# cornellius-gp/linear_operator

Measured on AMD Instinct MI355X. Metric: cg_member_matvecs_per_sec, higher is better.
Workload: dtype f32

## Files before the change

### linear_operator_amd/csrc/lo_rspace3.hip

```cpp
#include <algorithm>
#include <atomic>
#include <mutex>
#include <type_traits>
#include <stdlib.h>

#include "lo_device.h"
#include "lo_internal.h"
#include "lo_cg_onchip.h"
#include "lo_group_reduce.h"
#include "lo_cg_close.h"
#include "lo_f64_lanes.h"

namespace lo {

namespace {

typedef float f32x4 __attribute__((ext_vector_type(4)));
typedef __attribute__((address_space(1))) const f32x4 g_cf4;
typedef __attribute__((address_space(1))) const float g_cf;
typedef __attribute__((address_space(1))) float g_f;
typedef __attribute__((address_space(1))) const char g_cc;
template <class T>
__device__ __forceinline__ T* opaque_uniform(T* p) {
  asm volatile("" : "+s"(p));
  return p;
}

constexpr int R3_TPB = 256;
constexpr int R3_ROWS = 1024;

struct PeerOut {
  float* buf[7];
  int n;
  long long member_off;
};
PeerOut g_peer_out = {{nullptr, nullptr, nullptr, nullptr, nullptr, nullptr, nullptr}, 0, 0};
std::mutex g_peer_mu;

__host__ __device__ constexpr int r3_np(int RC) { return 2 * RC + 6; }

__device__ __forceinline__ unsigned xor4_dpp_u(unsigned x) {
  const int a = __builtin_amdgcn_update_dpp(0, (int)x, 0x104, 0xf, 0x5, false);
  return (unsigned)__builtin_amdgcn_update_dpp(a, (int)x, 0x114, 0xf, 0xa, false);
}
__device__ __forceinline__ double halve4_d(double lo, double hi, int lane) {
  const bool up = (lane & 4) != 0;
  const double keep = up ? hi : lo;
  const double send = up ? lo : hi;
  return keep + mk_d(xor4_dpp_u(lo_w(send)), xor4_dpp_u(hi_w(send)));
}

template <int CH>
__device__ __forceinline__ double rows_reduce_d(double (&p)[CH], int lane) {
  if constexpr (CH == 8) {
#pragma unroll
    for (int m = 0; m < 4; ++m) p[m] = halve4_d(p[m], p[m + 4], lane);
    p[0] = halve_pair_d<2>(p[0], p[2], lane);
    p[1] = halve_pair_d<2>(p[1], p[3], lane);
    return halve_pair_d<1>(p[0], p[1], lane);
  } else if constexpr (CH == 4) {
    p[0] = halve_pair_d<2>(p[0], p[2], lane);
    p[1] = halve_pair_d<2>(p[1], p[3], lane);
    return halve_pair_d<1>(p[0], p[1], lane);
  } else {
    return halve_pair_d<1>(p[0], p[1], lane);
  }
}

template <int RC, int GW>
__global__ __launch_bounds__(R3_TPB, 2) void k_cg_rspace3(OnchipArgs a, PeerOut po) {
  constexpr int CH = RC / 4;
  constexpr int RPI = 64 / CH;
  constexpr int NI = 256 / RPI;
  constexpr int NP = r3_np(RC);
  constexpr int MLD = RC + 2;
  constexpr int NH = RC / 2;
  constexpr int NG = 2 * GW * NP;
  __shared__ __attribute__((aligned(16))) float bst[4][256];
  __shared__ __attribute__((aligned(16))) float dst[4][256];
  __shared__ __attribute__((aligned(16))) double mat_s[3 * RC * MLD];
  __shared__ __attribute__((aligned(16))) double red[4][NP];
  __shared__ __attribute__((aligned(16))) double res[NP];
  __shared__ __attribute__((aligned(16))) double gv[4][32];
  __shared__ unsigned polw[GW > 1 ? NG : 2];
  const GroupPlace gp = group_place(GW, (int)gridDim.x / 8);
  if (!gp.active) return;
  const int grp = gp.grp, wig = gp.wig, ngroups = gp.ngroups;
  const int t = threadIdx.x, lane = t & 63, wave = t >> 6;
  const int wave_u = __builtin_amdgcn_readfirstlane(wave);
  unsigned long long* const gbase = a.gbuf + (size_t)grp * 2 * NG;
  unsigned tag = a.tag_base;
  bool same_xcd = false;
  const unsigned xcc = xcc_id();
  bool first = true;
  const int row0 = wig * R3_ROWS + 256 * wave_u;
  const int row0c = max(0, min(row0, a.N - 256));
  const bool di_full = a.dinv_mode == LO_DIAG_FULL;
  float* const bw = bst[wave_u];
  float* const dw = dst[wave_u];
  constexpr int NPF = 8;
  f32x4 pre[NPF];
  constexpr int NXT = NI - NPF;
  f32x4 nxt[NXT > 0 ? NXT : 1];
  auto request = [&](int64_t bm, int tl_, int i_lo, auto cnt, f32x4* dst) {
    const int ln_ = tl_ & 63, k_ = ln_ & (CH - 1), g_ = ln_ / CH;
    const unsigned loff = (unsigned)((g_ * RC + 4 * k_) * sizeof(float));
    g_cc* Cw = (g_cc*)(a.C + ((size_t)bm * a.N + row0c) * RC);
#pragma unroll
    for (int q = 0; q < decltype(cnt)::value / 8; ++q) {
      g_cc* bq = opaque_uniform(Cw + (i_lo + 8 * q + 4) * 1024);
#pragma unroll
      for (int i = 0; i < 8; ++i) dst[8 * q + i] = *(g_cf4*)(bq + loff + (i - 4) * 1024);
    }
  };
  int closed = 0;
  int64_t b = grp;
  {
    int tl0 = t;
    asm volatile("" : "+v"(tl0));
    if (b < a.B) {
      request(b, tl0, 0, std::integral_constant<int, NPF>{}, pre);
      request(b, tl0, NPF, std::integral_constant<int, NXT>{}, nxt);
    } else {
#pragma unroll
      for (int i = 0; i < NPF; ++i) pre[i] = (f32x4){0.f, 0.f, 0.f, 0.f};
    }
  }
  while (b < a.B) {
    const bool stamp = a.dbg && b == a.dbg_member && wig == 0 && t == 0;
    if (stamp) a.dbg[0] = wall_clock64();
    int drawn = 0;
    if (wig == 0 && t == 0) drawn = atomicAdd(a.next_member, 1);
    int tl = t;
    asm volatile("" : "+v"(tl));
    const int ln = tl & 63, k = ln & (CH - 1), g = ln / CH;
    f32x4 Cr[NI];
#pragma unroll
    for (int i = 0; i < NPF; ++i) Cr[i] = pre[i];
#pragma unroll
    for (int i = 0; i < NXT; ++i) Cr[NPF + i] = nxt[i];
    float bq4[4], dq4[4];
    {
      g_cf* bb_ = opaque_uniform((g_cf*)(a.rhs + (size_t)b * a.N + row0c));
      g_cf* dd_ = opaque_uniform((g_cf*)(di_full ? a.dinv + (size_t)b * a.N + row0c : a.dinv + b));
      const int lo_e = row0 - row0c, hi_e = max(0, min(256, a.N - row0c));
      const int dstride = di_full ? 1 : 0;
#pragma unroll
      for (int m = 0; m < 4; ++m) {
        const int e = ln + 64 * m;
        const bool own = e >= lo_e && e < hi_e;
        bq4[m] = own ? bb_[e] : 0.f;
        dq4[m] = own ? dd_[e * dstride] : 0.f;
      }
    }
    constexpr int NM = (3 * RC * RC / 2 + R3_TPB - 1) / R3_TPB;
    f32x4 mv[NM];
    {
      typedef __attribute__((address_space(1))) const f32x4 g_m4;
      const g_m4* src = (const g_m4*)(a.RSD + (size_t)b * 6 * RC * RC);
#pragma unroll
      for (int u = 0; u < NM; ++u) {
        const int e = min(tl + R3_TPB * u, 3 * RC * RC / 2 - 1);
        const int ms = e / (RC * RC / 2);
        const int mg = ms == 0 ? 0 : ms + 1;
        mv[u] = src[(size_t)mg * (RC * RC / 2) + (e - ms * (RC * RC / 2))];
      }
    }
    const double lam_mine = a.RSD[((size_t)b * 6 + 5) * RC * RC + min(ln & 31, RC - 1)];
#pragma unroll
    for (int m = 0; m < 4; ++m) {
      bw[ln + 64 * m] = bq4[m];
      dw[ln + 64 * m] = dq4[m];
    }
#pragma unroll
    for (int u = 0; u < NM; ++u) {
      const int e = tl + R3_TPB * u;
      if (e < 3 * RC * RC / 2) {
        const int mi = e / (RC / 2), jj = e % (RC / 2);
        *reinterpret_cast<f32x4*>(&mat_s[mi * MLD + 2 * jj]) = mv[u];
      }
    }
    __builtin_amdgcn_wave_barrier();
    if (stamp) a.dbg[1] = wall_clock64();

    {
      double aw[4] = {0.0, 0.0, 0.0, 0.0}, au[4] = {0.0, 0.0, 0.0, 0.0};
#pragma unroll
      for (int i0 = 0; i0 < NI; i0 += 4) {
#pragma unroll
        for (int i = i0; i < i0 + 4; ++i) {
          const int r = RPI * i + g;
          const double bb = (double)bw[r];
          const double bd = bb * (double)dw[r];
          const double c0 = (double)Cr[i].x, c1 = (double)Cr[i].y, c2 = (double)Cr[i].z, c3 = (double)Cr[i].w;
          aw[0] = fma(c0, bd, aw[0]); au[0] = fma(c0, bb, au[0]);
          aw[1] = fma(c1, bd, aw[1]); au[1] = fma(c1, bb, au[1]);
          aw[2] = fma(c2, bd, aw[2]); au[2] = fma(c2, bb, au[2]);
          aw[3] = fma(c3, bd, aw[3]); au[3] = fma(c3, bb, au[3]);
        }
        __builtin_amdgcn_sched_barrier(0);
      }
      double s_acc = 0.0, a_acc = 0.0, d2_acc = 0.0;
#pragma unroll
      for (int j = 0; j < 4; ++j) {
        const int rw = 64 * j + RPI * k + g;
        const double bb = (double)bw[rw], di = (double)dw[rw];
        s_acc = fma(bb, bb * di, s_acc);
        a_acc = fma(bb, bb, a_acc);
        d2_acc = fma(di, di, d2_acc);
      }
      double h0 = halve_pair_d<32>(aw[0], au[0], ln), h1 = halve_pair_d<32>(aw[1], au[1], ln);
      double h2 = halve_pair_d<32>(aw[2], au[2], ln), h3 = halve_pair_d<32>(aw[3], au[3], ln);
      h0 = halve_pair_d<16>(h0, h2, ln);
      h1 = halve_pair_d<16>(h1, h3, ln);
      double mine = halve_pair_d<8>(h0, h1, ln);
      if constexpr (CH <= 4) mine = bfly_add_d<4>(mine);
      if constexpr (CH <= 2) mine = bfly_add_d<2>(mine);
      const int comp = (((ln >> 4) & 1) << 1) | ((ln >> 3) & 1);
      const bool writer = (ln & 7 & ~(CH - 1)) == 0;
      if (writer) red[wave_u][((ln >> 5) ? RC : 0) + 4 * k + comp] = mine;
      const double ssum = wave_sum_fast_d(s_acc), asum = wave_sum_fast_d(a_acc), d2sum = wave_sum_fast_d(d2_acc);
      if (ln == 0) {
        red[wave_u][2 * RC] = ssum;
        red[wave_u][2 * RC + 1] = asum;
        red[wave_u][2 * RC + 2] = (wig == 0 && wave_u == 0) ? (double)(ngroups + drawn) : 0.0;
        red[wave_u][2 * RC + 3] = d2sum;
        unsigned xc = xcc;
        asm volatile("" : "+s"(xc));
        red[wave_u][2 * RC + 4] = (first && wave_u == 0) ? (double)xc : 0.0;
        red[wave_u][2 * RC + 5] = (first && wave_u == 0) ? (double)(xc * xc) : 0.0;
      }
    }
#pragma unroll
    for (int i = 0; i < NI; ++i) asm volatile("" : "+v"(Cr[i]));
    __builtin_amdgcn_sched_barrier(0);
    if (a.prefetch & 4) __builtin_amdgcn_s_setprio(3);
    {
      ++tag;
      int tt = (int)threadIdx.x;
      asm volatile("" : "+v"(tt));
      __syncthreads();
      if constexpr (GW == 1) {
        if (tt < NP) res[tt] = (red[0][tt] + red[1][tt]) + (red[2][tt] + red[3][tt]);
      } else {
        unsigned long long* slot = gbase + (size_t)(tag & 1u) * NG;
        if (tt < NP) {
          const double v = (red[0][tt] + red[1][tt]) + (red[2][tt] + red[3][tt]);
          unsigned long long* mine = slot + ((size_t)wig * NP + tt) * 2;
          granule_store(mine, granule_pack_bits(tag, lo_w(v)), same_xcd);
          granule_store(mine + 1, granule_pack_bits(tag, hi_w(v)), same_xcd);
        }
        constexpr int PER = (NG + R3_TPB - 1) / R3_TPB;
        constexpr int CKQ = PER < 8 ? PER : 8;
        unsigned spin = 0;
        bool lost = false;
#pragma unroll 1
        for (int q0 = 0; q0 < PER && !lost; q0 += CKQ) {
          unsigned long long x[CKQ];
          for (;;) {
            bool ok = true;
#pragma unroll
            for (int q = 0; q < CKQ; ++q) {
              const int idx = tt + R3_TPB * (q0 + q);
              x[q] = granule_load(slot + min(idx, NG - 1));
              ok = ok && (granule_tag(x[q]) == tag);
            }
            if (ok) break;
            if (poll_give_up(spin, a.err)) {
              lost = true;
              break;
            }
            __builtin_amdgcn_s_sleep(1);
          }
#pragma unroll
          for (int q = 0; q < CKQ; ++q) {
            const int idx = tt + R3_TPB * (q0 + q);
            if (idx < NG) polw[idx] = granule_bits(x[q]);
          }
        }
        __syncthreads();
        if (tt < NP) {
          double tot = 0.0;
#pragma unroll
          for (int w = 0; w < GW; ++w) tot += mk_d(polw[(w * NP + tt) * 2], polw[(w * NP + tt) * 2 + 1]);
          res[tt] = tot;
        }
      }
      __syncthreads();
    }
    if (GW > 1 && first) {
      unsigned xc = xcc;
      asm volatile("" : "+s"(xc));
      same_xcd = same_xcd_verdict(res[2 * RC + 4], res[2 * RC + 5], GW, xc, a.allow_l2_handoff);
    }
    first = false;
    if (stamp) a.dbg[2] = wall_clock64();
    const int64_t b_next = (int64_t)res[2 * RC + 2];
    {
      int tp = t;
      asm volatile("" : "+v"(tp));
      if (b_next < a.B) {
        request(b_next, tp, 0, std::integral_constant<int, NPF>{}, pre);
      } else {
#pragma unroll
        for (int i = 0; i < NPF; ++i) pre[i] = (f32x4){0.f, 0.f, 0.f, 0.f};
      }
    }
    if (a.prefetch & 1) __builtin_amdgcn_s_setprio(3);

    const int j = lane & 31, hf = lane >> 5;
    const bool live = j < RC;
    const int jr = live ? j : RC - 1;
    double yj = 0.0, xi = 0.0;
    float nrm;
    {
      double a0 = res[2 * RC + 1], s = res[2 * RC];
      const double d2 = res[2 * RC + 3];
      nrm = sqrtf((float)a0);
      const bool rhs_zero = nrm < a.eps;
      if (rhs_zero) nrm = 1.0f;
      const double inv = 1.0 / (double)nrm;
      const double w0 = live ? res[jr] * inv : 0.0, u0 = live ? res[RC + jr] * inv : 0.0;
      s *= inv * inv;
      a0 *= inv * inv;
      float sa = a.stop_after;
      asm volatile("" : "+s"(sa));
      const double sure_rz = 2.0 * (double)sa * (double)sa * sqrt(d2);
      auto own_row_dot = [&](const double* mrow, const double* vec) {
        double a0_ = 0.0, a1_ = 0.0;
#pragma unroll
        for (int q = 0; q < NH; q += 2) {
          const double2 xa = *reinterpret_cast<const double2*>(mrow + q);
          const double2 xx = *reinterpret_cast<const double2*>(vec + q);
          a0_ = fma(xa.x, xx.x, a0_);
          a1_ = fma(xa.y, xx.y, a1_);
        }
        double lo_, up_;
        halves_d(a0_ + a1_, lo_, up_);
        return lo_ + up_;
      };
      double* myv = gv[wave];
      if (hf == 0) myv[j] = w0;
      __builtin_amdgcn_wave_barrier();
      const double* row0m = mat_s + (size_t)jr * MLD + hf * NH;
      double c0 = own_row_dot(row0m, myv + hf * NH);
      double e0 = own_row_dot(row0m + (size_t)1 * RC * MLD, myv + hf * NH);
      const double* nrow = row0m + (size_t)2 * RC * MLD;
      const double* tucol = mat_s + (size_t)(1 * RC + hf * NH) * MLD + jr;
      c0 = live ? c0 : 0.0;
      e0 = live ? e0 : 0.0;
      double tau2 = s - lanes32_sum_d(c0 * e0);
      tau2 = tau2 > 0.0 ? tau2 : 0.0;
      const bool delicate = !rhs_zero && tau2 < 1e-2 * s;
      const double lam = live ? lam_mine : 1.0;
      long long ts_a = 0, ts_b = 0;
      if (stamp) ts_a = wall_clock64();
      double cj = c0, qj = 0.0, etaj = 0.0;
      double cp = 1.0, qp = 0.0, etap = 0.0;
      double rz = 0.0, pApE = 0.0, alpha = 0.0, beta = 0.0;
      float rn = 0.f, last_alpha = 0.f;
      bool conv = false;
      unsigned close_flags = 0u;
      const size_t bc = (size_t)b;
      const bool rec = wig == 0 && lane == 0;
      const int last_owner = (a.iters - 1) & 3;
      for (int kk = -1; kk < a.iters; ++kk) {
        if (kk >= 0) {
          last_alpha = (float)alpha;
          etaj = fma(alpha, qj, etaj);
          etap = fma(alpha, qp, etap);
          cj = fma(-alpha * lam, qj, cj);
          cp = fma(-alpha, qp, cp);
        }
        const double lc = lam * cj;
        const bool lo_h = hf == 0;
        const float inv_rz = __builtin_amdgcn_rcpf((float)rz);
        const double red2 = row16_sum_d(halve_pair_d<16>(lo_h ? cj * cj : lc * qj, lo_h ? lc * cj : 0.0, lane));
        const auto pick = [&](double v, int ln_) {
          return mk_d((unsigned)__builtin_amdgcn_readlane((int)lo_w(v), ln_),
                      (unsigned)__builtin_amdgcn_readlane((int)hi_w(v), ln_));
        };
        const double cc = pick(red2, 0), clc = pick(red2, 16), clq = pick(red2, 32);
        const double rzn = fma(cp * cp, tau2, cc);
        const bool sure = rzn > sure_rz;
        const bool rec_first = kk == 0 && a.close_gran == nullptr && wave == 0;
        const bool rec_last = kk == a.iters - 1 && wave == last_owner;
        const bool own = rec_first || rec_last || !sure;
        float rnn = 0.f;
        if (kk < 0) {
          const float s1f = (float)a0;
          rnn = __builtin_amdgcn_sqrtf(s1f < 0.f ? 0.f : s1f);
        } else if (own) {
          const double dl = fma(-cp, c0, cj);
          __builtin_amdgcn_wave_barrier();
          if (hf == 0) myv[j] = dl;
          __builtin_amdgcn_wave_barrier();
          double gj_;
          {
            double a0_ = 0.0, a1_ = 0.0;
#pragma unroll
            for (int q = 0; q < NH; q += 2) {
              const double2 dd = *reinterpret_cast<const double2*>(myv + hf * NH + q);
              a0_ = fma(tucol[(size_t)q * MLD], dd.x, a0_);
              a1_ = fma(tucol[(size_t)(q + 1) * MLD], dd.y, a1_);
            }
            double lo_, up_;
            halves_d(a0_ + a1_, lo_, up_);
            gj_ = live ? lo_ + up_ : 0.0;
          }
          __builtin_amdgcn_wave_barrier();
          if (hf == 0) myv[j] = gj_;
          __builtin_amdgcn_wave_barrier();
          const double nd = own_row_dot(nrow, myv + hf * NH);
          const double r2 = row16_sum_d(halve_pair_d<16>(gj_ * nd, gj_ * u0, lane));
          const double dnd = pick(r2, 0), dm = pick(r2, 16);
          const double s1 = fma(cp, fma(cp, a0, 2.0 * dm), dnd);
          const float s1f = (float)s1;
          rnn = __builtin_amdgcn_sqrtf(s1f < 0.f ? 0.f : s1f);
        }
        if (kk >= 0) {
          beta = ((float)rz < a.eps) ? 0.0 : (double)((float)rzn * inv_rz);
          if (rhs_zero) rnn = 0.f;
          rn = rnn;
          if (rec && (rec_first || rec_last)) a.resid_rec[(size_t)kk * a.B + bc] = rn;
        } else {
          beta = 0.0;
          rn = rnn;
          if (wig == 0 && t == 0) a.init_conv[bc] = (rn < a.stop_after) ? 1 : 0;
          close_flags = ((rn < a.stop_after) ? 1u : 0u) | (delicate ? 4u : 0u);
          if (delicate && rec && wave == 0) atomicOr(a.err + 4, 1);
        }
        if (kk == 0 && (rnn != rnn || rzn != rzn)) close_flags |= 2u;
        conv = (own || rhs_zero) ? (rn < a.stop_after) : false;
        rz = rzn;
        pApE = fma(beta, fma(beta, pApE, 2.0 * clq), clc);
        qj = fma(beta, qj, cj);
        qp = fma(beta, qp, cp);
        const double pAp = fma(qp * qp, tau2, pApE);
        alpha = ((float)pAp < a.eps) ? 0.0 : (double)((float)rz * __builtin_amdgcn_rcpf((float)pAp));
        if (conv) alpha = 0.0;
      }
      if (stamp) ts_b = wall_clock64();
      if (rec && wave == last_owner) {
        a.rhs_norm[bc] = nrm;
        a.rhs_is_zero[bc] = rhs_zero ? 1 : 0;
        a.rz[bc] = (float)rz;
        a.alpha[bc] = last_alpha;
        a.beta[bc] = (float)beta;
        a.resid_norm[bc] = rn;
        a.has_conv[bc] = conv ? 1 : 0;
        if (a.close_gran) {
          granule_store(a.close_gran + b, granule_pack(a.close_epoch | close_flags, rn), false);
        }
      }
      __builtin_amdgcn_wave_barrier();
      if (hf == 0) myv[j] = fma(-etap, e0, etaj);
      __builtin_amdgcn_wave_barrier();
      xi = etap;
      {
        const double* col = mat_s + (size_t)(hf * NH) * MLD + jr;
        double a0_ = 0.0, a1_ = 0.0;
#pragma unroll
        for (int q = 0; q < NH; q += 2) {
          const double2 ee = *reinterpret_cast<const double2*>(myv + hf * NH + q);
          a0_ = fma(col[(size_t)q * MLD], ee.x, a0_);
          a1_ = fma(col[(size_t)(q + 1) * MLD], ee.y, a1_);
        }
        double lo_, up_;
        halves_d(a0_ + a1_, lo_, up_);
        yj = lo_ + up_;
      }
      yj = live ? yj : 0.0;
      if (stamp) {
        a.dbg[5] = ts_a - a.dbg[2];
        a.dbg[6] = ts_b - ts_a;
        a.dbg[7] = wall_clock64() - ts_b;
      }
      __builtin_amdgcn_wave_barrier();
      if (hf == 0) myv[j] = yj * (double)nrm;
      __builtin_amdgcn_wave_barrier();
    }
    if (a.close_gran && wig == 0 && po.n == 0 && __builtin_amdgcn_readfirstlane((int)(b_next >= a.B))) {
      int tc = (int)threadIdx.x;
      asm volatile("" : "+v"(tc));
      cg_close_solve(a, ngroups, tc);
      closed = 1;
#pragma unroll
      for (int i = 0; i < NPF; ++i) pre[i] = (f32x4){0.f, 0.f, 0.f, 0.f};
    }
    if (!(a.prefetch & 2)) __builtin_amdgcn_s_setprio(0);
    if (stamp) a.dbg[3] = wall_clock64();
    {
      int l2 = lane;
      asm volatile("" : "+v"(l2));
      const int k2 = l2 & (CH - 1), g2 = l2 / CH;
      const double* myv = gv[wave];
      const double2 ya = *reinterpret_cast<const double2*>(&myv[4 * k2]);
      const double2 yb = *reinterpret_cast<const double2*>(&myv[4 * k2 + 2]);
      g_f* const xb = opaque_uniform((g_f*)(a.xout + (size_t)b * a.N + row0c));
      const bool more = b_next < a.B;
      g_cc* const Cn = (g_cc*)(a.C + ((size_t)(more ? b_next : b) * a.N + row0c) * RC);
      const unsigned loffn = (unsigned)((g2 * RC + 4 * k2) * sizeof(float));
#pragma unroll
      for (int js = 0; js < 4; ++js) {
        constexpr int J0 = NPF / CH;
        const int jj = (js + J0) & 3;
        double p[CH];
#pragma unroll
        for (int m = 0; m < CH; ++m) {
          const f32x4 c4 = Cr[CH * jj + m];
          p[m] = fma((double)c4.w, yb.y, fma((double)c4.z, yb.x, fma((double)c4.y, ya.y, (double)c4.x * ya.x)));
        }
        const double xv = rows_reduce_d<CH>(p, l2);
        const int rw = 64 * jj + RPI * k2 + g2;
        const int row = row0c + rw;
        const double acc = fma(xi, (double)bw[rw], xv);
        if (row >= row0 && row < a.N) {
          const float xval = (float)(acc * (double)dw[rw]);
          xb[rw] = xval;
          for (int pp = 0; pp < po.n; ++pp)
            ((g_f*)po.buf[pp])[((size_t)(b + po.member_off)) * a.N + row] = xval;
        }
        if (CH * jj >= NPF) {
          g_cc* bqn = opaque_uniform(Cn + (CH * jj + 4) * 1024);
#pragma unroll
          for (int m = 0; m < CH; ++m)
            nxt[CH * jj - NPF + m] = more ? *(g_cf4*)(bqn + loffn + (m - 4) * 1024) : (f32x4){0.f, 0.f, 0.f, 0.f};
        }
      }
      __builtin_amdgcn_wave_barrier();
    }
    __builtin_amdgcn_s_setprio(0);
    if (stamp) a.dbg[4] = wall_clock64();
    __syncthreads();
    b = b_next;
  }
  if (a.close_gran && wig == 0 && !closed) {
    int te = (int)threadIdx.x;
    asm volatile("" : "+v"(te));
    cg_close_solve(a, ngroups, te);
  }
}

int rspace3_prio() {
  static const int prio = [] {
    const char* e = getenv("LO_RS_PRIO");
    return e ? atoi(e) : 3;
  }();
  return prio;
}

constexpr size_t HO_MAX_WGS = 2 * 320;
constexpr size_t HO_GRAN_PER_WG = 432;
constexpr size_t HO_MAX_MEMBERS = 65536;
constexpr size_t HO_HEAD_BYTES = 256;
constexpr unsigned HO_TAG_LIMIT = 0xfff00000u;
constexpr unsigned HO_EPOCH_LIMIT = 0x1ffffff0u;
struct HandoffBlock {
  char* buf = nullptr;
  size_t bytes = 0;
  bool failed = false;
  unsigned next_tag = 1, next_epoch = 1;
  unsigned last_launch = 0;
  std::atomic<unsigned> confirmed{0};
  bool force_clear = false;
  unsigned clears = 0, launches = 0;
};
HandoffBlock g_handoff[16];
std::atomic<unsigned> g_handoff_ids{0};

HandoffBlock* handoff_block() {
  int dev = 0;
  if (hipGetDevice(&dev) != hipSuccess || dev < 0 || dev >= 16) return nullptr;
  HandoffBlock& h = g_handoff[dev];
  if (!h.buf && !h.failed) {
    h.bytes = HO_HEAD_BYTES + (HO_MAX_WGS * HO_GRAN_PER_WG + HO_MAX_MEMBERS) * sizeof(unsigned long long);
    if (hipMalloc(&h.buf, h.bytes) != hipSuccess || hipMemset(h.buf, 0, h.bytes) != hipSuccess) {
      (void)hipGetLastError();
      h.buf = nullptr;
      h.failed = true;
    }
  }
  return h.buf ? &h : nullptr;
}

bool handoff_advance(unsigned* next_tag, unsigned* next_epoch, int64_t B, unsigned* tag_base, unsigned* epoch) {
  bool wrap = false;
  const unsigned need = (unsigned)B + 2u;
  if (*next_tag >= HO_TAG_LIMIT - need || *next_epoch >= HO_EPOCH_LIMIT) {
    *next_tag = 1;
    *next_epoch = 1;
    wrap = true;
  }
  *tag_base = *next_tag;
  *epoch = *next_epoch;
  *next_tag += need;
  *next_epoch += 1;
  return wrap;
}

struct OwnedLaunch {
  bool inject;
  unsigned* launch_id;
};

template <int RC, int GW>
int rspace3_go(const OnchipArgs& a, int nwg, const OwnedLaunch* own, hipStream_t st) {
  int per_cu = 0;
  if (LO_OCCUPANCY_CACHED(per_cu, (k_cg_rspace3<RC, GW>), R3_TPB, 0) != hipSuccess || per_cu < 2) return LO_ERR_UNSUPPORTED;
  LO_PROF_BEGIN("cg_onchip", st);
  ResidentLaunch guard(st);
  OnchipArgs a2 = a;
  a2.prefetch = rspace3_prio();
  if (own) {
    hipStreamCaptureStatus cap = hipStreamCaptureStatusNone;
    if (hipStreamIsCapturing(st, &cap) != hipSuccess || cap != hipStreamCaptureStatusNone) {
      (void)hipGetLastError();
      return LO_ERR_UNSUPPORTED;
    }
    HandoffBlock* h = (a.B <= (int64_t)HO_MAX_MEMBERS && (size_t)2 * nwg <= HO_MAX_WGS) ? handoff_block() : nullptr;
    if (!h) return LO_ERR_UNSUPPORTED;
    bool clear = h->force_clear || h->last_launch != h->confirmed.load(std::memory_order_acquire);
    h->force_clear = false;
    clear = handoff_advance(&h->next_tag, &h->next_epoch, a.B, &a2.tag_base, &a2.close_epoch) || clear;
    h->last_launch = g_handoff_ids.fetch_add(1, std::memory_order_relaxed) + 1;
    if (h->last_launch == 0) h->last_launch = g_handoff_ids.fetch_add(1, std::memory_order_relaxed) + 1;
    *own->launch_id = h->last_launch;
    ++h->launches;
    if (clear) {
      ++h->clears;
      const int zrc = zero_span(h->buf, h->bytes, st);
      if (zrc) return zrc;
    }
    a2.close_epoch <<= 3;
    a2.handoff_owned = 1;
    a2.err = reinterpret_cast<int*>(h->buf);
    a2.next_member = a2.err + 1;
    a2.close_count = a2.err + 2;
    a2.gbuf = reinterpret_cast<unsigned long long*>(h->buf + HO_HEAD_BYTES);
    a2.close_gran = a2.gbuf + HO_MAX_WGS * HO_GRAN_PER_WG;
    if (own->inject) LO_HIP_CHECK(hipMemsetAsync(a2.err, 1, 1, st));
  }
  PeerOut po;
  {
    std::lock_guard<std::mutex> lk(g_peer_mu);
    po = g_peer_out;
  }
  hipLaunchKernelGGL((k_cg_rspace3<RC, GW>), dim3(2 * nwg), dim3(R3_TPB), 0, st, a2, po);
  LO_PROF_END(st);
  LO_LAUNCH_CHECK();
  return LO_OK;
}

template <int RC>
int rspace3_gw(const OnchipArgs& a, int nwg, const OwnedLaunch* own, hipStream_t st) {
  switch (a.GW) {
    case 1: return rspace3_go<RC, 1>(a, nwg, own, st);
    case 2: return rspace3_go<RC, 2>(a, nwg, own, st);
    case 4: return rspace3_go<RC, 4>(a, nwg, own, st);
    case 8: return rspace3_go<RC, 8>(a, nwg, own, st);
    case 16: return rspace3_go<RC, 16>(a, nwg, own, st);
    case 32: return rspace3_go<RC, 32>(a, nwg, own, st);
  }
  return LO_ERR_UNSUPPORTED;
}

int rspace3_dispatch(int RC, const OnchipArgs& a, int nwg, const OwnedLaunch* own, hipStream_t st) {
  if (!a.RSD || a.x || a.c != 1 || a.ab_rec || !a.xout || a.GW > 32 || a.N < 256 || (int64_t)a.GW * R3_ROWS < a.N)
    return LO_ERR_UNSUPPORTED;
  if (RC == 32) return rspace3_gw<32>(a, nwg, own, st);
  if (RC == 16) return rspace3_gw<16>(a, nwg, own, st);
  if (RC == 8) return rspace3_gw<8>(a, nwg, own, st);
  return LO_ERR_UNSUPPORTED;
}

}

int rspace3_launch(int RC, const OnchipArgs& a, int nwg, hipStream_t st) { return rspace3_dispatch(RC, a, nwg, nullptr, st); }

int rspace3_launch_owned(int RC, const OnchipArgs& a, int nwg, bool inject, unsigned* launch_id, hipStream_t st) {
  if (!a.close_gran || !a.close_ctrl || !a.close_mirror || a.dbg) return LO_ERR_UNSUPPORTED;
  const OwnedLaunch own = {inject, launch_id};
  return rspace3_dispatch(RC, a, nwg, &own, st);
}

void handoff_launch_confirm(unsigned launch_id) {
  int dev = 0;
  if (hipGetDevice(&dev) != hipSuccess || dev < 0 || dev >= 16) return;
  g_handoff[dev].confirmed.store(launch_id, std::memory_order_release);
}

}

extern "C" int lo_peer_gather_set(float* const* bufs, int n, long long member_offset) {
  if (n < 0 || n > 7 || (n > 0 && !bufs)) return LO_ERR_BADARG;
  std::lock_guard<std::mutex> lk(lo::g_peer_mu);
  for (int i = 0; i < 7; ++i) lo::g_peer_out.buf[i] = i < n ? bufs[i] : nullptr;
  lo::g_peer_out.n = n;
  lo::g_peer_out.member_off = member_offset;
  return LO_OK;
}

extern "C" int lo_resident_handoff_debug(int32_t force_clear, int64_t set_next_tag, int64_t set_next_epoch, uint32_t* out) {
  lo::ResidentLock guard;
  int dev = 0;
  if (hipGetDevice(&dev) != hipSuccess || dev < 0 || dev >= 16) return LO_ERR_BADARG;
  lo::HandoffBlock& h = lo::g_handoff[dev];
  if (set_next_tag > 0xffffffffll || set_next_epoch > 0xffffffffll) return LO_ERR_BADARG;
  if (set_next_tag >= 0) h.next_tag = (unsigned)set_next_tag;
  if (set_next_epoch >= 0) h.next_epoch = (unsigned)set_next_epoch;
  if (force_clear) h.force_clear = true;
  if (out) {
    out[0] = h.next_tag;
    out[1] = h.next_epoch;
    out[2] = h.clears;
    out[3] = h.launches;
  }
  return LO_OK;
}
```

Before: 37.16 million.

## Prefetch next member's rhs/dinv and defer matrix LDS stores past projection

The rhs and diagonal-inverse loads for the next CG member are now issued during the previous member's output phase, so they no longer sit on the critical path at loop start. The RSD matrix stores into LDS move after the projection reduction and become branch-free, with out-of-range lanes writing to a padding slot. The prefetch of the next C tile is made unconditional by zeroing the offset when there is no next member, which removes a select. The change also adds debug-stamp selection by workgroup and an opaque offset on the member atomic. In exchange it holds extra registers live across the iteration and risks stale values when no next member exists.

```diff
diff --git a/linear_operator_amd/csrc/lo_rspace3.hip b/linear_operator_amd/csrc/lo_rspace3.hip
--- a/linear_operator_amd/csrc/lo_rspace3.hip
+++ b/linear_operator_amd/csrc/lo_rspace3.hip
@@ -78,7 +78,7 @@
   constexpr int NG = 2 * GW * NP;
   __shared__ __attribute__((aligned(16))) float bst[4][256];
   __shared__ __attribute__((aligned(16))) float dst[4][256];
-  __shared__ __attribute__((aligned(16))) double mat_s[3 * RC * MLD];
+  __shared__ __attribute__((aligned(16))) double mat_s[3 * RC * MLD + 2];
   __shared__ __attribute__((aligned(16))) double red[4][NP];
   __shared__ __attribute__((aligned(16))) double res[NP];
   __shared__ __attribute__((aligned(16))) double gv[4][32];
@@ -113,24 +113,46 @@
       for (int i = 0; i < 8; ++i) dst[8 * q + i] = *(g_cf4*)(bq + loff + (i - 4) * 1024);
     }
   };
+  float bn4[4], dn4[4];
+  auto request_bd = [&](int64_t bm, int tl_) {
+    const int ln_ = tl_ & 63;
+    g_cf* bb_ = opaque_uniform((g_cf*)(a.rhs + (size_t)bm * a.N + row0c));
+    g_cf* dd_ = opaque_uniform((g_cf*)(di_full ? a.dinv + (size_t)bm * a.N + row0c : a.dinv + bm));
+    const int lo_e = row0 - row0c, hi_e = max(0, min(256, a.N - row0c));
+    const int dstride = di_full ? 1 : 0;
+#pragma unroll
+    for (int m = 0; m < 4; ++m) {
+      const int e = ln_ + 64 * m;
+      const bool own = e >= lo_e && e < hi_e;
+      bn4[m] = own ? bb_[e] : 0.f;
+      dn4[m] = own ? dd_[e * dstride] : 0.f;
+    }
+  };
   int closed = 0;
   int64_t b = grp;
   {
     int tl0 = t;
     asm volatile("" : "+v"(tl0));
     if (b < a.B) {
+      request_bd(b, tl0);
       request(b, tl0, 0, std::integral_constant<int, NPF>{}, pre);
       request(b, tl0, NPF, std::integral_constant<int, NXT>{}, nxt);
     } else {
 #pragma unroll
       for (int i = 0; i < NPF; ++i) pre[i] = (f32x4){0.f, 0.f, 0.f, 0.f};
+#pragma unroll
+      for (int m = 0; m < 4; ++m) bn4[m] = dn4[m] = 0.f;
     }
   }
   while (b < a.B) {
-    const bool stamp = a.dbg && b == a.dbg_member && wig == 0 && t == 0;
+    const bool stamp = a.dbg && b == (a.dbg_member & 0xfffff) && wig == (a.dbg_member >> 20) && t == 0;
     if (stamp) a.dbg[0] = wall_clock64();
     int drawn = 0;
-    if (wig == 0 && t == 0) drawn = atomicAdd(a.next_member, 1);
+    if (wig == 0 && t == 0) {
+      int zo = 0;
+      asm volatile("" : "+v"(zo));
+      drawn = atomicAdd(a.next_member + zo, 1);
+    }
     int tl = t;
     asm volatile("" : "+v"(tl));
     const int ln = tl & 63, k = ln & (CH - 1), g = ln / CH;
@@ -139,20 +161,6 @@
     for (int i = 0; i < NPF; ++i) Cr[i] = pre[i];
 #pragma unroll
     for (int i = 0; i < NXT; ++i) Cr[NPF + i] = nxt[i];
-    float bq4[4], dq4[4];
-    {
-      g_cf* bb_ = opaque_uniform((g_cf*)(a.rhs + (size_t)b * a.N + row0c));
-      g_cf* dd_ = opaque_uniform((g_cf*)(di_full ? a.dinv + (size_t)b * a.N + row0c : a.dinv + b));
-      const int lo_e = row0 - row0c, hi_e = max(0, min(256, a.N - row0c));
-      const int dstride = di_full ? 1 : 0;
-#pragma unroll
-      for (int m = 0; m < 4; ++m) {
-        const int e = ln + 64 * m;
-        const bool own = e >= lo_e && e < hi_e;
-        bq4[m] = own ? bb_[e] : 0.f;
-        dq4[m] = own ? dd_[e * dstride] : 0.f;
-      }
-    }
     constexpr int NM = (3 * RC * RC / 2 + R3_TPB - 1) / R3_TPB;
     f32x4 mv[NM];
     {
@@ -169,16 +177,8 @@
     const double lam_mine = a.RSD[((size_t)b * 6 + 5) * RC * RC + min(ln & 31, RC - 1)];
 #pragma unroll
     for (int m = 0; m < 4; ++m) {
-      bw[ln + 64 * m] = bq4[m];
-      dw[ln + 64 * m] = dq4[m];
-    }
-#pragma unroll
-    for (int u = 0; u < NM; ++u) {
-      const int e = tl + R3_TPB * u;
-      if (e < 3 * RC * RC / 2) {
-        const int mi = e / (RC / 2), jj = e % (RC / 2);
-        *reinterpret_cast<f32x4*>(&mat_s[mi * MLD + 2 * jj]) = mv[u];
-      }
+      bw[ln + 64 * m] = bn4[m];
+      dw[ln + 64 * m] = dn4[m];
     }
     __builtin_amdgcn_wave_barrier();
     if (stamp) a.dbg[1] = wall_clock64();
@@ -233,6 +233,14 @@
     }
 #pragma unroll
     for (int i = 0; i < NI; ++i) asm volatile("" : "+v"(Cr[i]));
+    __builtin_amdgcn_sched_barrier(0);
+#pragma unroll
+    for (int u = 0; u < NM; ++u) {
+      const int e = tl + R3_TPB * u;
+      const int mi = e / (RC / 2), jj = e % (RC / 2);
+      const int at = e < 3 * RC * RC / 2 ? mi * MLD + 2 * jj : 3 * RC * MLD;
+      *reinterpret_cast<f32x4*>(&mat_s[at]) = mv[u];
+    }
     __builtin_amdgcn_sched_barrier(0);
     if (a.prefetch & 4) __builtin_amdgcn_s_setprio(3);
     {
@@ -499,8 +507,10 @@
       const double2 yb = *reinterpret_cast<const double2*>(&myv[4 * k2 + 2]);
       g_f* const xb = opaque_uniform((g_f*)(a.xout + (size_t)b * a.N + row0c));
       const bool more = b_next < a.B;
-      g_cc* const Cn = (g_cc*)(a.C + ((size_t)(more ? b_next : b) * a.N + row0c) * RC);
-      const unsigned loffn = (unsigned)((g2 * RC + 4 * k2) * sizeof(float));
+      const int64_t bn = more ? b_next : b;
+      request_bd(bn, l2);
+      g_cc* const Cn = (g_cc*)(a.C + ((size_t)bn * a.N + row0c) * RC);
+      const unsigned loffn = more ? (unsigned)((g2 * RC + 4 * k2) * sizeof(float)) : 0u;
 #pragma unroll
       for (int js = 0; js < 4; ++js) {
         constexpr int J0 = NPF / CH;
@@ -525,7 +535,7 @@
           g_cc* bqn = opaque_uniform(Cn + (CH * jj + 4) * 1024);
 #pragma unroll
           for (int m = 0; m < CH; ++m)
-            nxt[CH * jj - NPF + m] = more ? *(g_cf4*)(bqn + loffn + (m - 4) * 1024) : (f32x4){0.f, 0.f, 0.f, 0.f};
+            nxt[CH * jj - NPF + m] = *(g_cf4*)(bqn + loffn + (m - 4) * 1024);
         }
       }
       __builtin_amdgcn_wave_barrier();
```

New measurement: 37.61 million, median of 6. About the same (+1.2%).

## Defer final-iteration residual norm computation into next member's load phase

Applied to the files above, without the earlier changes.

The last CG iteration's residual-norm computation for a member is deferred. Its inputs are stashed in shared memory, and the norm is computed and written at the start of the next member's iteration, overlapping with the loads. The end-of-member __syncthreads is moved to after the deferred block. The change also alters the polling chunk size for the group reduction and preloads matrix columns into registers before the final matvec. Correctness now depends on res and mat_s still holding the previous member's values when the deferred work runs, which looks fragile.

```diff
diff --git a/linear_operator_amd/csrc/lo_rspace3.hip b/linear_operator_amd/csrc/lo_rspace3.hip
--- a/linear_operator_amd/csrc/lo_rspace3.hip
+++ b/linear_operator_amd/csrc/lo_rspace3.hip
@@ -65,6 +65,53 @@
   } else {
     return halve_pair_d<1>(p[0], p[1], lane);
   }
+}
+
+__device__ __forceinline__ double pick_d(double v, int ln_) {
+  return mk_d((unsigned)__builtin_amdgcn_readlane((int)lo_w(v), ln_), (unsigned)__builtin_amdgcn_readlane((int)hi_w(v), ln_));
+}
+template <int NH>
+__device__ __forceinline__ double own_row_dot(const double* mrow, const double* vec) {
+  double a0_ = 0.0, a1_ = 0.0;
+#pragma unroll
+  for (int q = 0; q < NH; q += 2) {
+    const double2 xa = *reinterpret_cast<const double2*>(mrow + q);
+    const double2 xx = *reinterpret_cast<const double2*>(vec + q);
+    a0_ = fma(xa.x, xx.x, a0_);
+    a1_ = fma(xa.y, xx.y, a1_);
+  }
+  double lo_, up_;
+  halves_d(a0_ + a1_, lo_, up_);
+  return lo_ + up_;
+}
+template <int NH, int MLD>
+__device__ __forceinline__ float resid_norm_c(double dl, double cp, double a0, double u0, bool live, int j, int hf, int lane,
+                                              double* vec, const double* tucol, const double* nrow) {
+  __builtin_amdgcn_wave_barrier();
+  if (hf == 0) vec[j] = dl;
+  __builtin_amdgcn_wave_barrier();
+  double gj_;
+  {
+    double a0_ = 0.0, a1_ = 0.0;
+#pragma unroll
+    for (int q = 0; q < NH; q += 2) {
+      const double2 dd = *reinterpret_cast<const double2*>(vec + hf * NH + q);
+      a0_ = fma(tucol[(size_t)q * MLD], dd.x, a0_);
+      a1_ = fma(tucol[(size_t)(q + 1) * MLD], dd.y, a1_);
+    }
+    double lo_, up_;
+    halves_d(a0_ + a1_, lo_, up_);
+    gj_ = live ? lo_ + up_ : 0.0;
+  }
+  __builtin_amdgcn_wave_barrier();
+  if (hf == 0) vec[j] = gj_;
+  __builtin_amdgcn_wave_barrier();
+  const double nd = own_row_dot<NH>(nrow, vec + hf * NH);
+  const double r2 = row16_sum_d(halve_pair_d<16>(gj_ * nd, gj_ * u0, lane));
+  const double dnd = pick_d(r2, 0), dm = pick_d(r2, 16);
+  const double s1 = fma(cp, fma(cp, a0, 2.0 * dm), dnd);
+  const float s1f = (float)s1;
+  return __builtin_amdgcn_sqrtf(s1f < 0.f ? 0.f : s1f);
 }
 
 template <int RC, int GW>
@@ -83,6 +130,7 @@
   __shared__ __attribute__((aligned(16))) double res[NP];
   __shared__ __attribute__((aligned(16))) double gv[4][32];
   __shared__ unsigned polw[GW > 1 ? NG : 2];
+  __shared__ __attribute__((aligned(16))) double late_v[32 + 4];
   const GroupPlace gp = group_place(GW, (int)gridDim.x / 8);
   if (!gp.active) return;
   const int grp = gp.grp, wig = gp.wig, ngroups = gp.ngroups;
@@ -114,6 +162,7 @@
     }
   };
   int closed = 0;
+  bool late_pending = false;
   int64_t b = grp;
   {
     int tl0 = t;
@@ -130,7 +179,7 @@
     const bool stamp = a.dbg && b == a.dbg_member && wig == 0 && t == 0;
     if (stamp) a.dbg[0] = wall_clock64();
     int drawn = 0;
-    if (wig == 0 && t == 0) drawn = atomicAdd(a.next_member, 1);
+    if (wig == 0 && t == 0) drawn = atomicAdd(opaque_uniform(a.next_member), 1);
     int tl = t;
     asm volatile("" : "+v"(tl));
     const int ln = tl & 63, k = ln & (CH - 1), g = ln / CH;
@@ -167,6 +216,40 @@
       }
     }
     const double lam_mine = a.RSD[((size_t)b * 6 + 5) * RC * RC + min(ln & 31, RC - 1)];
+    if (late_pending && wave_u == ((a.iters - 1) & 3)) {
+      int l3 = lane;
+      asm volatile("" : "+v"(l3));
+      const int j = l3 & 31, hf = l3 >> 5;
+      const bool live = j < RC;
+      const int jr = live ? j : RC - 1;
+      double a0 = res[2 * RC + 1];
+      float nrm = sqrtf((float)a0);
+      const bool rhs_zero = nrm < a.eps;
+      if (rhs_zero) nrm = 1.0f;
+      const double inv = 1.0 / (double)nrm;
+      const double u0 = live ? res[RC + jr] * inv : 0.0;
+      a0 *= inv * inv;
+      const double* tucol = mat_s + (size_t)(1 * RC + hf * NH) * MLD + jr;
+      const double* nrow = mat_s + (size_t)(2 * RC + jr) * MLD + hf * NH;
+      const double dl = late_v[j], cp = late_v[32];
+      const unsigned flags0 = (unsigned)late_v[33];
+      const size_t bp = (size_t)late_v[34];
+      float rn = resid_norm_c<NH, MLD>(dl, cp, a0, u0, live, j, hf, l3, late_v, tucol, nrow);
+      if (rhs_zero) rn = 0.f;
+      if (l3 == 0) {
+        int it = a.iters;
+        long long nb = a.B;
+        asm volatile("" : "+s"(it), "+s"(nb));
+        const unsigned close_flags = flags0 | ((it == 1 && rn != rn) ? 2u : 0u);
+        a.resid_rec[(size_t)(it - 1) * (size_t)nb + bp] = rn;
+        a.resid_norm[bp] = rn;
+        a.has_conv[bp] = (rn < a.stop_after) ? 1 : 0;
+        if (a.close_gran) {
+          granule_store(a.close_gran + bp, granule_pack(a.close_epoch | close_flags, rn), false);
+        }
+      }
+    }
+    __syncthreads();
 #pragma unroll
     for (int m = 0; m < 4; ++m) {
       bw[ln + 64 * m] = bq4[m];
@@ -251,7 +334,8 @@
           granule_store(mine + 1, granule_pack_bits(tag, hi_w(v)), same_xcd);
         }
         constexpr int PER = (NG + R3_TPB - 1) / R3_TPB;
-        constexpr int CKQ = PER < 8 ? PER : 8;
+        constexpr int CKQ = GW == 32 ? 8 : PER <= 9 ? PER : (PER + 1) / 2;
+        static_assert(CKQ <= 9 && 2 * CKQ >= (GW == 32 ? 16 : PER), "poll rounds");
         unsigned spin = 0;
         bool lost = false;
 #pragma unroll 1
@@ -326,25 +410,12 @@
       float sa = a.stop_after;
       asm volatile("" : "+s"(sa));
       const double sure_rz = 2.0 * (double)sa * (double)sa * sqrt(d2);
-      auto own_row_dot = [&](const double* mrow, const double* vec) {
-        double a0_ = 0.0, a1_ = 0.0;
-#pragma unroll
-        for (int q = 0; q < NH; q += 2) {
-          const double2 xa = *reinterpret_cast<const double2*>(mrow + q);
-          const double2 xx = *reinterpret_cast<const double2*>(vec + q);
-          a0_ = fma(xa.x, xx.x, a0_);
-          a1_ = fma(xa.y, xx.y, a1_);
-        }
-        double lo_, up_;
-        halves_d(a0_ + a1_, lo_, up_);
-        return lo_ + up_;
-      };
       double* myv = gv[wave];
       if (hf == 0) myv[j] = w0;
       __builtin_amdgcn_wave_barrier();
       const double* row0m = mat_s + (size_t)jr * MLD + hf * NH;
-      double c0 = own_row_dot(row0m, myv + hf * NH);
-      double e0 = own_row_dot(row0m + (size_t)1 * RC * MLD, myv + hf * NH);
+      double c0 = own_row_dot<NH>(row0m, myv + hf * NH);
+      double e0 = own_row_dot<NH>(row0m + (size_t)1 * RC * MLD, myv + hf * NH);
       const double* nrow = row0m + (size_t)2 * RC * MLD;
       const double* tucol = mat_s + (size_t)(1 * RC + hf * NH) * MLD + jr;
       c0 = live ? c0 : 0.0;
@@ -364,6 +435,8 @@
       const size_t bc = (size_t)b;
       const bool rec = wig == 0 && lane == 0;
       const int last_owner = (a.iters - 1) & 3;
+      const bool late = wig == 0 && a.iters > 0 && wave_u == last_owner &&
+                        __builtin_amdgcn_readfirstlane((int)(b_next < a.B)) != 0;
       for (int kk = -1; kk < a.iters; ++kk) {
         if (kk >= 0) {
           last_alpha = (float)alpha;
@@ -376,53 +449,34 @@
         const bool lo_h = hf == 0;
         const float inv_rz = __builtin_amdgcn_rcpf((float)rz);
         const double red2 = row16_sum_d(halve_pair_d<16>(lo_h ? cj * cj : lc * qj, lo_h ? lc * cj : 0.0, lane));
-        const auto pick = [&](double v, int ln_) {
-          return mk_d((unsigned)__builtin_amdgcn_readlane((int)lo_w(v), ln_),
-                      (unsigned)__builtin_amdgcn_readlane((int)hi_w(v), ln_));
-        };
-        const double cc = pick(red2, 0), clc = pick(red2, 16), clq = pick(red2, 32);
+        const double cc = pick_d(red2, 0), clc = pick_d(red2, 16), clq = pick_d(red2, 32);
         const double rzn = fma(cp * cp, tau2, cc);
         const bool sure = rzn > sure_rz;
         const bool rec_first = kk == 0 && a.close_gran == nullptr && wave == 0;
-        const bool rec_last = kk == a.iters - 1 && wave == last_owner;
+        const bool rec_last = kk == a.iters - 1 && wave == last_owner && wig == 0;
+        const bool late_now = late && kk == a.iters - 1;
         const bool own = rec_first || rec_last || !sure;
         float rnn = 0.f;
         if (kk < 0) {
           const float s1f = (float)a0;
           rnn = __builtin_amdgcn_sqrtf(s1f < 0.f ? 0.f : s1f);
+        } else if (late_now) {
+          const double dl = fma(-cp, c0, cj);
+          if (hf == 0) late_v[j] = dl;
+          if (lane == 0) late_v[32] = cp;
         } else if (own) {
           const double dl = fma(-cp, c0, cj);
-          __builtin_amdgcn_wave_barrier();
-          if (hf == 0) myv[j] = dl;
-          __builtin_amdgcn_wave_barrier();
-          double gj_;
-          {
-            double a0_ = 0.0, a1_ = 0.0;
-#pragma unroll
-            for (int q = 0; q < NH; q += 2) {
-              const double2 dd = *reinterpret_cast<const double2*>(myv + hf * NH + q);
-              a0_ = fma(tucol[(size_t)q * MLD], dd.x, a0_);
-              a1_ = fma(tucol[(size_t)(q + 1) * MLD], dd.y, a1_);
-            }
-            double lo_, up_;
-            halves_d(a0_ + a1_, lo_, up_);
-            gj_ = live ? lo_ + up_ : 0.0;
-          }
-          __builtin_amdgcn_wave_barrier();
-          if (hf == 0) myv[j] = gj_;
-          __builtin_amdgcn_wave_barrier();
-          const double nd = own_row_dot(nrow, myv + hf * NH);
-          const double r2 = row16_sum_d(halve_pair_d<16>(gj_ * nd, gj_ * u0, lane));
-          const double dnd = pick(r2, 0), dm = pick(r2, 16);
-          const double s1 = fma(cp, fma(cp, a0, 2.0 * dm), dnd);
-          const float s1f = (float)s1;
-          rnn = __builtin_amdgcn_sqrtf(s1f < 0.f ? 0.f : s1f);
+          rnn = resid_norm_c<NH, MLD>(dl, cp, a0, u0, live, j, hf, lane, myv, tucol, nrow);
         }
         if (kk >= 0) {
           beta = ((float)rz < a.eps) ? 0.0 : (double)((float)rzn * inv_rz);
           if (rhs_zero) rnn = 0.f;
           rn = rnn;
-          if (rec && (rec_first || rec_last)) a.resid_rec[(size_t)kk * a.B + bc] = rn;
+          if (rec && (rec_first || rec_last) && !late_now) {
+            long long nb = a.B;
+            asm volatile("" : "+s"(nb));
+            a.resid_rec[(size_t)kk * (size_t)nb + bc] = rn;
+          }
         } else {
           beta = 0.0;
           rn = rnn;
@@ -447,10 +501,15 @@
         a.rz[bc] = (float)rz;
         a.alpha[bc] = last_alpha;
         a.beta[bc] = (float)beta;
-        a.resid_norm[bc] = rn;
-        a.has_conv[bc] = conv ? 1 : 0;
-        if (a.close_gran) {
-          granule_store(a.close_gran + b, granule_pack(a.close_epoch | close_flags, rn), false);
+        if (late) {
+          late_v[33] = (double)close_flags;
+          late_v[34] = (double)b;
+        } else {
+          a.resid_norm[bc] = rn;
+          a.has_conv[bc] = conv ? 1 : 0;
+          if (a.close_gran) {
+            granule_store(a.close_gran + b, granule_pack(a.close_epoch | close_flags, rn), false);
+          }
         }
       }
       __builtin_amdgcn_wave_barrier();
@@ -459,12 +518,20 @@
       xi = etap;
       {
         const double* col = mat_s + (size_t)(hf * NH) * MLD + jr;
+        double cv[NH];
+        double2 ee[NH / 2];
+#pragma unroll
+        for (int q = 0; q < NH; q += 2) {
+          ee[q / 2] = *reinterpret_cast<const double2*>(myv + hf * NH + q);
+          cv[q] = col[(size_t)q * MLD];
+          cv[q + 1] = col[(size_t)(q + 1) * MLD];
+        }
+        __builtin_amdgcn_sched_barrier(0);
         double a0_ = 0.0, a1_ = 0.0;
 #pragma unroll
         for (int q = 0; q < NH; q += 2) {
-          const double2 ee = *reinterpret_cast<const double2*>(myv + hf * NH + q);
-          a0_ = fma(col[(size_t)q * MLD], ee.x, a0_);
-          a1_ = fma(col[(size_t)(q + 1) * MLD], ee.y, a1_);
+          a0_ = fma(cv[q], ee[q / 2].x, a0_);
+          a1_ = fma(cv[q + 1], ee[q / 2].y, a1_);
         }
         double lo_, up_;
         halves_d(a0_ + a1_, lo_, up_);
@@ -532,7 +599,7 @@
     }
     __builtin_amdgcn_s_setprio(0);
     if (stamp) a.dbg[4] = wall_clock64();
-    __syncthreads();
+    late_pending = wig == 0 && a.iters > 0 && __builtin_amdgcn_readfirstlane((int)(b_next < a.B)) != 0;
     b = b_next;
   }
   if (a.close_gran && wig == 0 && !closed) {
```

New measurement: 36.85 million before, 37.76 million after (median of 6 runs). +2.5%, better.
